# marvinli00/genie2

Hardware: AMD Instinct MI355X
Metric: denoise-steps/sec (N=256, T=1000, batch=8) (higher is better)
Workload: dtype f32 (pair-stack products as 3 f16 MFMAs on 2xf16-split operands, f32 accumulate); 1 GPU; unconditional N=256, T=1000, batch=8 per GPU, random-init base Denoiser (15.7M params), scale=0.6, reverse-loop steps 995..676; parallelism=replica per GPU x1, no data-path collective

## Files before the change

### genie2_amd/csrc/common.h

```cpp
#pragma once
#include <hip/hip_runtime.h>
#include <stdint.h>
#include "../../include/genie_hip.h"

typedef float f32x16 __attribute__((ext_vector_type(16)));
typedef float f32x4 __attribute__((ext_vector_type(4)));

#define GENIE_LN_EPS 1e-5f

#ifdef __HIPCC__

__device__ __forceinline__ f32x16 mfma_8k(const float4 a, const float4 b, f32x16 c) {
    c = __builtin_amdgcn_mfma_f32_32x32x2f32(a.x, b.x, c, 0, 0, 0);
    c = __builtin_amdgcn_mfma_f32_32x32x2f32(a.y, b.y, c, 0, 0, 0);
    c = __builtin_amdgcn_mfma_f32_32x32x2f32(a.z, b.z, c, 0, 0, 0);
    c = __builtin_amdgcn_mfma_f32_32x32x2f32(a.w, b.w, c, 0, 0, 0);
    return c;
}

__device__ __forceinline__ f32x16 zero16() {
    f32x16 z;
#pragma unroll
    for (int i = 0; i < 16; ++i) z[i] = 0.f;
    return z;
// ... 145 lines not shown
};
struct StructLayerW {
    float *proj_w, *proj_b;
    float *head_w;
    float *out_w, *out_b;
    float *ln_ipa_g, *ln_ipa_b;
    float *t1_w, *t1_b, *t2_w, *t2_b, *t3_w, *t3_b;
    float *ln_tr_g, *ln_tr_b;
    float *bb_w, *bb_b;
};

struct HxGemmW { const float* w; const unsigned char* img; float inv_s; };

struct genie_train_ws;
struct genie_ctx {
    genie_dims_t d;
    genie_train_ws* train;
    int device;
    char err[512];

    bool have_weights;
    float* wdev;
    bool hx;
    unsigned char* hxdev;
    HxGemmW hxg[128]; int n_hxg;
    unsigned hx_launches;
    size_t wdev_floats;
    float *single_w;
    float *pij_w;
    float *relpos_t;
    float *templ_w;
    float *motif_w;
    float *ipa_bias_w, *ipa_bias_b;
    PairLayerW* pair;
    StructLayerW* st;

    bool have_tables;
    float *pos_tab, *chain_tab, *t_tab, *sched;
    int n_pos, n_chain;
    float* sched_host;

    int B, N, NP;
    bool have_feats, has_motif;
    int32_t *f_aatype, *f_rmask, *f_ridx, *f_cidx;
    float *f_pos;
    uint8_t *f_fsm, *f_fstm, *f_ifm;
    float *rmaskf;

    void* ws; size_t ws_bytes;
    float *p, *acm, *bcm, *xcm, *pstatic, *ipa_bias;
    float *spart;
    unsigned *pmax;
    float *xsingle, *s0, *s, *s1, *s2, *h1, *h2, *pij, *proj, *cat;
    float *kT, *v, *qp, *kpT, *vp;
    float *vf, *vmax;
    float *ta_tb, *ta_xn, *ta_qkvg;
    float *rots_w, *trans_w;
    int32_t* tsteps;
    float *loop_z;

    bool prof;
    struct ProfRec { int cls; hipEvent_t a, b; };
    ProfRec* prof_recs; int prof_n, prof_cap;
    double prof_ms[KC_COUNT]; int64_t prof_cnt[KC_COUNT];
    double train_gemm_flop;

// ... 46 lines not shown
```

### genie2_amd/csrc/genie_api.hip

```cpp
#include <stdio.h>
#include <stdlib.h>
#include <string.h>
#include <math.h>
#include <algorithm>
#include <cmath>
#include <new>
#include <string>
#include <vector>

#include "common.h"

void pair_kernels_init();
void pair_fused_kernels_init();
void single_kernels_init(const genie_dims_t& d, int n_max);
void launch_scale_copy(genie_ctx* h, hipStream_t st, const float* in, float* out, int n, float s);
size_t ipa_attn_lds(const genie_dims_t& d, int N);

static char g_create_err[512] = "";

void set_handle_free_error(const char* msg) { snprintf(g_create_err, sizeof g_create_err, "%s", msg); }

#define SET_ERR(h, ...) do { snprintf((h)->err, sizeof((h)->err), __VA_ARGS__); } while (0)
#define HIP_TRY(h, call) do { hipError_t e_ = (call); if (e_ != hipSuccess) { \
    SET_ERR(h, "%s failed: %s (%s:%d)", #call, hipGetErrorString(e_), __FILE__, __LINE__); return GENIE_E_HIP; } } while (0)
// ... 365 lines not shown
            };
            A.sq = scale_of(q_w); A.sk = scale_of(k_w); A.sv = scale_of(v_w);
        }
        const size_t nh = (size_t)d.pair_transition_n * cp;
        const float* lg = c.take(cp); const float* lb = c.take(cp);
        const float* w1 = c.take(nh * cp); const float* b1 = c.take(nh);
        const float* w2 = c.take(cp * nh); const float* b2 = c.take(cp);
        {
            std::vector<float> w1v(w1, w1 + nh * cp), b1v(b1, b1 + nh);
            fold_ln(w1v, b1v, (int)nh, (int)cp, lg, lb);
            slot(&L.pt_ln_g, ones_off); slot(&L.pt_ln_b, zeros_off);
            slot(&L.pt_w1, img.pack(w1v.data(), (int)nh, (int)cp)); slot(&L.pt_b1, img.raw(b1v.data(), nh));
            HxTransW& X = L.hx_pt;
            const float s1 = p2floor(16384.0 / max_abs(w1v.data(), nh * cp)), s2 = p2floor(16384.0 / max_abs(w2, cp * nh));
            const float sh = p2floor(32768.0 / hx_bound(w1v.data(), b1v.data(), (int)nh, (int)cp));
            X.sx = HX_SX; X.c1 = sh / (HX_SX * s1); X.c2 = 1.0f / (sh * s2);
            hxfix.push_back({&X.img, hx.begin()});
            for (size_t hb = 0; hb < nh / 32; ++hb) {
                for (int kc = 0; kc < 8; ++kc)
                    hx.unit([&](int i, int hh, int e) { return w1v[(32 * hb + i) * cp + 16 * kc + 8 * hh + e] * s1; });
                for (int cc = 0; cc < 2; ++cc)
                    for (int ob = 0; ob < 4; ++ob)
                        hx.unit([&](int j, int hh, int e) {
                            return w2[(size_t)(32 * ob + j) * nh + 32 * hb + 16 * cc + (e & 3) + 8 * (e >> 2) + 4 * hh] * s2; });
            }
            std::vector<float> b1s(nh), b2s(cp);
            for (size_t r = 0; r < nh; ++r) b1s[r] = b1v[r] * HX_SX * s1;
            for (size_t r = 0; r < cp; ++r) b2s[r] = b2[r] * sh * s2;
            slot(&X.b1s, img.raw(b1s.data(), nh)); slot(&X.b2s, img.raw(b2s.data(), cp));
            pt_save[l] = PtSave{w1v, std::vector<float>(w2, w2 + cp * nh), s1, s2};
        }
        slot(&L.pt_w2, img.pack(w2, (int)cp, (int)nh)); slot(&L.pt_b2, img.raw(b2, cp));
    }
    {
        auto ck = [](int kc, int hh, int e) { return 16 * kc + (e & 3) + 8 * (e >> 2) + 4 * hh; };
        auto emit_O = [&](const TmSave& t) {
            for (int which = 0; which < 2; ++which)
                for (int st = 0; st < 2; ++st)
                    for (int obl = 0; obl < 2; ++obl)
                        for (int kc = 0; kc < 8; ++kc) {
                            const std::vector<float>& m = which == 0 ? t.zw : t.gw;
                            const float sc = which == 0 ? t.szo : t.sgo;
                            const size_t ob = 2 * st + obl;
                            hx.unit([&](int i, int hh, int e) { return m[(32 * ob + i) * cp + ck(kc, hh, e)] * sc; });
                        }
        };
        auto emit_T = [&](const PtSave& t) {
            const size_t nh = (size_t)d.pair_transition_n * cp;
            for (size_t hb = 0; hb < nh / 32; ++hb) {
                for (int kc = 0; kc < 8; ++kc)
                    hx.unit([&](int i, int hh, int e) { return t.w1v[(32 * hb + i) * cp + ck(kc, hh, e)] * t.s1; });
                for (int cc = 0; cc < 2; ++cc)
                    for (int ob = 0; ob < 4; ++ob)
                        hx.unit([&](int j, int hh, int e) { return t.w2[(size_t)(32 * ob + j) * nh + 32 * hb + ck(cc, hh, e)] * t.s2; });
            }
        };
        auto emit_P = [&](const TmSave& t) {
            for (size_t pass = 0; pass < 8; ++pass)
                for (int kc = 0; kc < 8; ++kc) {
                    hx.unit([&](int i, int hh, int e) { return t.w[(32 * pass + i) * cp + ck(kc, hh, e)] * t.sp; });
                    hx.unit([&](int i, int hh, int e) { return t.w[(2 * ch + 32 * pass + i) * cp + ck(kc, hh, e)] * t.sg; });
                }
        };
        for (int l = 0; l < d.n_pair_transform_layer; ++l) {
            hxfix.push_back({&h->pair[l].fa.img, hx.begin()});
            emit_O(tm_save[2 * l]); emit_P(tm_save[2 * l + 1]);
            hxfix.push_back({&h->pair[l].fb.img, hx.begin()});
            emit_O(tm_save[2 * l + 1]); emit_T(pt_save[l]);
            if (l + 1 < d.n_pair_transform_layer) emit_P(tm_save[2 * l + 2]);
        }
    }
    const size_t H = d.n_head_ipa, C = d.c_hidden_ipa, Pq = d.n_qk_point, Pv = d.n_v_point;
    const size_t ncat = ipa_cat_n(d);
    std::vector<float> wb_all, bb_all;
    for (int l = 0; l < d.n_structure_layer; ++l) {
        StructLayerW& S = h->st[l];
        const float* hw = c.take(H);
        const float* q_w = c.take(H * C * cs);            const float* q_b = c.take(H * C);
        const float* kv_w = c.take(2 * H * C * cs);       const float* kv_b = c.take(2 * H * C);
        const float* qp_w = c.take(3 * H * Pq * cs);      const float* qp_b = c.take(3 * H * Pq);
        const float* kp_w = c.take(3 * H * (Pq + Pv) * cs); const float* kp_b = c.take(3 * H * (Pq + Pv));
        const float* b_w = c.take(H * cp);                const float* b_b = c.take(H);
        const float* o_w = c.take(cs * ncat);             const float* o_b = c.take(cs);
        const float* li_g = c.take(cs); const float* li_b = c.take(cs);
        const float* t1w = c.take(cs * cs); const float* t1b = c.take(cs);
        const float* t2w = c.take(cs * cs); const float* t2b = c.take(cs);
        const float* t3w = c.take(cs * cs); const float* t3b = c.take(cs);
        const float* lt_g = c.take(cs); const float* lt_b = c.take(cs);
        const float* bw = c.take(6 * cs); const float* bbs = c.take(6);
        if (!bbs) { SET_ERR(h, "genie_load_weights: blob too short"); return GENIE_E_ARG; }
        slot(&S.head_w, img.raw(hw, H));
        auto w = vcat({{q_w, H * C * cs}, {kv_w, 2 * H * C * cs}, {qp_w, 3 * H * Pq * cs}, {kp_w, 3 * H * (Pq + Pv) * cs}});
        auto bv = vcat({{q_b, H * C}, {kv_b, 2 * H * C}, {qp_b, 3 * H * Pq}, {kp_b, 3 * H * (Pq + Pv)}});
        pack_gemm(&S.proj_w, w.data(), ipa_proj_n(d), (int)cs);
        slot(&S.proj_b, img.raw(bv.data(), bv.size()));
        wb_all.insert(wb_all.end(), b_w, b_w + H * cp);
        bb_all.insert(bb_all.end(), b_b, b_b + H);
        pack_gemm(&S.out_w, o_w, (int)cs, (int)ncat); slot(&S.out_b, img.raw(o_b, cs));
        slot(&S.ln_ipa_g, img.raw(li_g, cs)); slot(&S.ln_ipa_b, img.raw(li_b, cs));
        pack_gemm(&S.t1_w, t1w, (int)cs, (int)cs); slot(&S.t1_b, img.raw(t1b, cs));
        pack_gemm(&S.t2_w, t2w, (int)cs, (int)cs); slot(&S.t2_b, img.raw(t2b, cs));
        pack_gemm(&S.t3_w, t3w, (int)cs, (int)cs); slot(&S.t3_b, img.raw(t3b, cs));
        slot(&S.ln_tr_g, img.raw(lt_g, cs)); slot(&S.ln_tr_b, img.raw(lt_b, cs));
        slot(&S.bb_w, img.raw(bw, 6 * cs)); slot(&S.bb_b, img.raw(bbs, 6));
    }
    pack_gemm(&h->ipa_bias_w, wb_all.data(), (int)(d.n_structure_layer * H), (int)cp);
    slot(&h->ipa_bias_b, img.raw(bb_all.data(), bb_all.size()));
    if (c.left != 0) { SET_ERR(h, "genie_load_weights: %zu floats left over", c.left); return GENIE_E_ARG; }

    if (h->wdev) { (void)hipFree(h->wdev); h->wdev = nullptr; }
    img.add(64);
    HIP_TRY(h, hipMalloc((void**)&h->wdev, img.data.size() * sizeof(float)));
    HIP_TRY(h, hipMemcpy(h->wdev, img.data.data(), img.data.size() * sizeof(float), hipMemcpyHostToDevice));
    h->wdev_floats = img.data.size();
    for (auto& f : fix) *f.first = h->wdev + f.second;
    if (h->hxdev) { (void)hipFree(h->hxdev); h->hxdev = nullptr; }
    hx.begin();
    HIP_TRY(h, hipMalloc((void**)&h->hxdev, hx.d.size() * 2 + 256));
    HIP_TRY(h, hipMemcpy(h->hxdev, hx.d.data(), hx.d.size() * 2, hipMemcpyHostToDevice));
    for (auto& f : hxfix) *f.first = h->hxdev + f.second;
    h->n_hxg = 0;
    const int hxg_cap = (int)(sizeof(h->hxg) / sizeof(h->hxg[0]));
    if ((int)gfix.size() > hxg_cap) { SET_ERR(h, "genie_load_weights: %zu row-GEMM weights exceed the %d hx image slots", gfix.size(), hxg_cap); return GENIE_E_ARG; }
    for (auto& g : gfix) h->hxg[h->n_hxg++] = HxGemmW{*g.slot, h->hxdev + g.hx_off, g.inv_s};
    h->have_weights = true;
    return GENIE_OK;
}

int genie_set_tables(genie_handle_t h, const float* pos_tab, int n_pos, const float* chain_tab, int n_chain,
                     const float* t_tab, const float* sched) {
    if (!h || !pos_tab || !chain_tab || !t_tab || !sched || n_pos < 1 || n_chain < 1) return GENIE_E_ARG;
    HIP_TRY(h, hipSetDevice(h->device));
    const genie_dims_t& d = h->d;
    const size_t T1 = d.n_timestep + 1;
    const size_t a = (size_t)n_pos * d.c_pos_emb, b = (size_t)n_chain * d.c_chain_emb, c = T1 * d.c_timestep_emb, s = 4 * T1;
    if (h->pos_tab) (void)hipFree(h->pos_tab);
    HIP_TRY(h, hipMalloc((void**)&h->pos_tab, (a + b + c + s) * sizeof(float)));
    h->chain_tab = h->pos_tab + a;
    h->t_tab = h->chain_tab + b;
    h->sched = h->t_tab + c;
// ... 77 lines not shown
    HIP_TRY(h, hipMemcpyAsync(h->f_ridx, f->residue_index, M * 4, hipMemcpyDeviceToDevice, st));
    HIP_TRY(h, hipMemcpyAsync(h->f_cidx, f->chain_index, M * 4, hipMemcpyDeviceToDevice, st));
    HIP_TRY(h, hipMemcpyAsync(h->f_fsm, f->fixed_sequence_mask, M, hipMemcpyDeviceToDevice, st));
    HIP_TRY(h, hipMemcpyAsync(h->f_fstm, f->fixed_structure_mask, P, hipMemcpyDeviceToDevice, st));
    HIP_TRY(h, hipMemcpyAsync(h->f_ifm, f->interface_mask, M, hipMemcpyDeviceToDevice, st));
    hipLaunchKernelGGL(k_mask_to_float, dim3((unsigned)((M + 255) / 256)), dim3(256), 0, st, h->f_rmask, h->rmaskf, (int)M);
    HIP_TRY(h, hipMemsetAsync(h->acm, 0, (size_t)B * cp * NP * NP * 4, st));
    HIP_TRY(h, hipMemsetAsync(h->vf, 0, ipa_vf_floats(d, B, N) * 4, st));
    HIP_TRY(h, hipMemsetAsync(h->bcm, 0, (size_t)B * cp * NP * NP * 4, st));
    single_kernels_init(d, N);
    {
        unsigned any = 0;
        HIP_TRY(h, hipMemsetAsync(h->pmax, 0, sizeof(unsigned), st));
        launch_any_nonzero(h, st, h->f_fstm, P, h->pmax);
        HIP_TRY(h, hipMemcpyAsync(&any, h->pmax, sizeof(unsigned), hipMemcpyDeviceToHost, st));
        HIP_TRY(h, hipStreamSynchronize(st));
        h->has_motif = any != 0;
    }
    launch_pair_static(h, st);
    HIP_TRY(h, hipGetLastError());
    h->have_feats = true;
    return GENIE_OK;
}

static int denoise_internal(genie_ctx* h, hipStream_t st, const float* trans, const float* rots, const int32_t* ts_dev,
                            const int8_t* codes, float* z_out, const genie_taps_t* taps) {
    const genie_dims_t& d = h->d;
    const int B = h->B, N = h->N, M = B * N;
    const size_t P = (size_t)M * N;
    const int cs = d.c_s, cp = d.c_p;
    const int ldx = (single_in(d) + 7) / 8 * 8;
    auto d2d = [&](void* dst, const void* src, size_t bytes) { return hipMemcpyAsync(dst, src, bytes, hipMemcpyDeviceToDevice, st); };

    h->hx_launches = 1;
    launch_scale_copy(h, st, trans, h->trans_w, M * 3, d.rescale);
    HIP_TRY(h, d2d(h->rots_w, rots, (size_t)M * 9 * 4));

    launch_single_input(h, st, ts_dev);
    launch_gemm_rows(h, st, h->xsingle, ldx, M, ldx, h->single_w, cs, nullptr, nullptr, 0, h->rmaskf, 0, h->s0, cs);
    if (taps && taps->s) HIP_TRY(h, d2d(taps->s, h->s0, (size_t)M * cs * 4));

    launch_gemm_rows(h, st, h->s0, cs, M, cs, h->pij_w, 2 * cp, nullptr, nullptr, 0, nullptr, 0, h->pij, 2 * cp);
    launch_pair_init(h, st, h->trans_w, h->rots_w, codes);
    if (taps && taps->p_init) HIP_TRY(h, d2d(taps->p_init, h->p, P * cp * 4));

    const bool fused = launch_pair_stack_fused(h, st, taps ? taps->p_trimul_out0 : nullptr, taps ? taps->p_layer0 : nullptr);
    for (int l = 0; l < (fused ? 0 : d.n_pair_transform_layer); ++l) {
        launch_trimul(h, st, h->pair[l].out, true);
        if (l == 0 && taps && taps->p_trimul_out0) HIP_TRY(h, d2d(taps->p_trimul_out0, h->p, P * cp * 4));
        launch_trimul(h, st, h->pair[l].in, false);
        if (d.n_head_tri > 0) {
            launch_triatt(h, st, h->pair[l].ta_start, true);
            launch_triatt(h, st, h->pair[l].ta_end, false);
            if (l == 0 && taps && taps->p_tri_att0) HIP_TRY(h, d2d(taps->p_tri_att0, h->p, P * cp * 4));
        }
        launch_pair_transition(h, st, h->pair[l]);
        if (l == 0 && taps && taps->p_layer0) HIP_TRY(h, d2d(taps->p_layer0, h->p, P * cp * 4));
    }
    if (taps && taps->p) HIP_TRY(h, d2d(taps->p, h->p, P * cp * 4));

    launch_ipa_bias(h, st);
    HIP_TRY(h, d2d(h->s, h->s0, (size_t)M * cs * 4));
    if (taps && taps->states) HIP_TRY(h, d2d(taps->states, h->s0, (size_t)M * cs * 4));
    int n_state = 1;
    const int nproj = ipa_proj_n(d), ncat = ipa_cat_n(d);
    bool split = h->st2 && B >= 2 && M >= 1024 && ipa_attn_splits(h) && !getenv("GENIE_NO_STRUCT_SPLIT");
// ... 228 lines not shown
```

### genie2_amd/csrc/hx_fused.h

```cpp
#pragma once
#include "hx_pair.h"

#define FZ_SB_BZ 0
#define FZ_SB_BG 128
#define FZ_SB_B1 256
#define FZ_SB_B2 768
#define FZ_SB_BP 896
#define FZ_SB_FLOATS 1408
#define FZ_OOR 0x7FFFFFF0
#define FZ_COMPILER_FENCE() asm volatile("" ::: "memory")

struct FusedArgs {
    float* z; const float* xcm; const float* rmask; const unsigned char* wimg;
    const float *bzs, *bgs, *b1s, *b2s, *bproj;
    unsigned *acm, *bcm;
    int N, NP, n_wtiles, n_hb;
    unsigned cm_bytes, z_bytes;
    float sx, cgo, cz, c1, c2, inv_c2, cpa, cpb, cg;
    int rev;
};

__device__ __forceinline__ void fz_zt_read(float4 (&raw)[16], const unsigned char* zt, int pl, int h, int half) {
#pragma unroll
    for (int q = 0; q < 4; ++q) {
        const int g = 4 * q + h;
        raw[2 * (4 * half + q)] = *reinterpret_cast<const float4*>(zt + pl * 256 + ((g ^ (pl & 15)) << 4));
        raw[2 * (4 * half + q) + 1] = *reinterpret_cast<const float4*>(zt + pl * 256 + (((g + 2) ^ (pl & 15)) << 4));
    }
}

__device__ __forceinline__ void fz_zt_chunk(float4& a, float4& b, const unsigned char* zt, int pl, int h, int q) {
    const int g = 4 * q + h;
    a = *reinterpret_cast<const float4*>(zt + pl * 256 + ((g ^ (pl & 15)) << 4));
    b = *reinterpret_cast<const float4*>(zt + pl * 256 + (((g + 2) ^ (pl & 15)) << 4));
}

__device__ __forceinline__ void fz_store_half(rsrc_t rz, unsigned char* zt, const f32x16& v0, const f32x16& v1, int lane, int soff,
                                              int row_stride, int nvalid, int hf) {
    const int pl = lane & 31, h = lane >> 5;
    FZ_COMPILER_FENCE();
#pragma unroll
    for (int q = 0; q < 4; ++q) {
        const f32x16& v = (q < 2) ? v0 : v1;
        const int r0 = 8 * (q & 1);
        const int g = 4 * q + h;
        *reinterpret_cast<float4*>(zt + pl * 256 + ((g ^ (pl & 15)) << 4)) = make_float4(v[r0], v[r0 + 1], v[r0 + 2], v[r0 + 3]);
        *reinterpret_cast<float4*>(zt + pl * 256 + (((g + 2) ^ (pl & 15)) << 4)) = make_float4(v[r0 + 4], v[r0 + 5], v[r0 + 6], v[r0 + 7]);
    }
    hx_lds_done();
#pragma unroll
    for (int j = 0; j < 8; ++j) {
        const int r = 4 * j + (lane >> 4);
// ... 36 lines not shown
```

### genie2_amd/csrc/pair_fused_kernels.hip

```cpp
#include <string.h>
#include "hx_fused.h"

#define FZ_LDS_BYTES (2 * HX_STAGE_BYTES + 6144 + 8 * HX_ZT_BYTES)

template <bool COL, bool HAS_T, bool HAS_P = true>
__global__ __launch_bounds__(512, 1) void k_pair_fused(const FusedArgs A) {
    extern __shared__ __attribute__((aligned(16))) unsigned char smb[];
    float* sb = reinterpret_cast<float*>(smb + 2 * HX_STAGE_BYTES);
    const int lane = threadIdx.x & 63, wave = UNI(threadIdx.x >> 6);
    const int h = lane >> 5, pl = lane & 31;
    const int N = A.N, NP = A.NP, n_wtiles = A.n_wtiles;
    const int ntile = (N + 31) >> 5;
    const int n_tiles = (n_wtiles + 7) / 8;
    const int rev = A.rev;
    const int n_hb = HAS_T ? A.n_hb : 0;
    const int PBASE = 4 + n_hb;
    const rsrc_t rw = hx_rsrc(A.wimg, (unsigned)((PBASE + (HAS_P ? 8 : 0)) * HX_STAGE_BYTES));
    const rsrc_t rx = hx_rsrc(A.xcm, A.cm_bytes), rz = hx_rsrc(A.z, A.z_bytes);
    const rsrc_t ra = hx_rsrc(A.acm, A.cm_bytes), rb = hx_rsrc(A.bcm, A.cm_bytes);
    const int lane16 = lane * 16;
    const int sstride = NP * NP * 4;
    const int zstride = COL ? N * 512 : 512;
    auto issue = [&](int s, int buf) {
        if (wave >= 4) {
#pragma unroll
            for (int q = 0; q < 8; ++q) {
                const int p = 8 * (wave - 4) + q;
                hx_dma(rw, smb + buf * HX_STAGE_BYTES + p * 1024, lane16, s * HX_STAGE_BYTES + p * 1024);
            }
        }
    };
    unsigned char* zt = smb + 2 * HX_STAGE_BYTES + 6144 + wave * HX_ZT_BYTES;
    auto tile_geom = [&](int tile, int& zsoff, int& nv, int& cmoff) {
        const int wt = min(HX_PHYS(tile) * 8 + wave, n_wtiles - 1);
        const int st = wt % ntile, line = (wt / ntile) % N, b = wt / (ntile * N);
        nv = min(32, N - st * 32);
        zsoff = COL ? ((b * N + st * 32) * N + line) * 512 : ((b * N + line) * N + st * 32) * 512;
        cmoff = ((b * 128 * NP + line) * NP + st * 32) * 4;
    };
    const int vx = (4 * h * NP * NP + pl) * 4;
#define FZ_XLOAD(c, xoff) do {                                                                                              \
        raw[2 * (c)].x = hx_load(rx, vx, (xoff) + (16 * (c) + 0) * sstride); raw[2 * (c)].y = hx_load(rx, vx, (xoff) + (16 * (c) + 1) * sstride); \
        raw[2 * (c)].z = hx_load(rx, vx, (xoff) + (16 * (c) + 2) * sstride); raw[2 * (c)].w = hx_load(rx, vx, (xoff) + (16 * (c) + 3) * sstride); \
        raw[2 * (c) + 1].x = hx_load(rx, vx, (xoff) + (16 * (c) + 8) * sstride); raw[2 * (c) + 1].y = hx_load(rx, vx, (xoff) + (16 * (c) + 9) * sstride); \
        raw[2 * (c) + 1].z = hx_load(rx, vx, (xoff) + (16 * (c) + 10) * sstride); raw[2 * (c) + 1].w = hx_load(rx, vx, (xoff) + (16 * (c) + 11) * sstride); \
    } while (0)

    int tile = blockIdx.x;
    issue(0, 0);
    for (int u = threadIdx.x; u < FZ_SB_FLOATS; u += 512) {
        float v = 0.f;
        if (u < FZ_SB_BG) v = A.bzs[u];
        else if (u < FZ_SB_B1) v = A.bgs[u - FZ_SB_BG];
        else if (u < FZ_SB_B2) { if (HAS_T && u - FZ_SB_B1 < n_hb * 32) v = A.b1s[u - FZ_SB_B1]; }
        else if (u < FZ_SB_BP) { if (HAS_T) v = A.b2s[u - FZ_SB_B2]; }
        else if (HAS_P) v = A.bproj[u - FZ_SB_BP];
        sb[u] = v;
    }
    float4 raw[16];
    {
        int zs, nv, cm;
        tile_geom(tile, zs, nv, cm);
        hx_zt_dma(rz, zt, lane, zs, zstride, nv, 1);
    }
    hx_stage_landed();
    __syncthreads();

#pragma unroll 1
    for (; tile < n_tiles; tile += gridDim.x) {
        const int wt_raw = HX_PHYS(tile) * 8 + wave;
        const bool act = wt_raw < n_wtiles;
        const int wt = act ? wt_raw : n_wtiles - 1;
        const int st = wt % ntile, line = (wt / ntile) % N, b = wt / (ntile * N);
        const int t0i = st * 32;
        const int nvalid = act ? min(32, N - t0i) : 0;
        int zsoff, znv, cmoff;
        tile_geom(tile, zsoff, znv, cmoff);
        int bo = 0;
        asm volatile("" : "+v"(bo));
        const float* sbt = sb + bo;
        int lane_t = lane;
        asm volatile("" : "+v"(lane_t));
        const int pl_t = lane_t & 31, h_t = lane_t >> 5;
#pragma unroll
        for (int c = 0; c < 8; ++c) FZ_XLOAD(c, cmoff);
        const float msk = (pl < nvalid) ? A.rmask[b * N + line] * A.rmask[b * N + t0i + pl] : 0.f;
        const bool more = tile + (int)gridDim.x < n_tiles;
        int n_zsoff = 0, n_nv = 1, n_cmoff = 0;
        if (more) tile_geom(tile + gridDim.x, n_zsoff, n_nv, n_cmoff);
        hx_vm_done();
        f32x16 v[4];

// ... 89 lines not shown
                    for (int q = 0; q < 4; ++q) fz_zt_chunk(res[2 * q], res[2 * q + 1], zt, pl_t, h_t, q);
                } else {
#pragma unroll
                    for (int q = 0; q < 8; ++q) res[q] = rz1[q];
                }
#pragma unroll
                for (int r = 0; r < 16; ++r) {
                    const float g0 = A.cz * __builtin_amdgcn_rcpf(1.0f + __builtin_amdgcn_exp2f(ga[r] * A.cgo));
                    const float g1 = A.cz * __builtin_amdgcn_rcpf(1.0f + __builtin_amdgcn_exp2f(gb[r] * A.cgo));
                    const float4 za = res[2 * (r >> 3) + ((r & 7) >> 2)], zb = res[2 * (2 + (r >> 3)) + ((r & 7) >> 2)];
                    const float z0 = (r & 3) == 0 ? za.x : (r & 3) == 1 ? za.y : (r & 3) == 2 ? za.z : za.w;
                    const float z1 = (r & 3) == 0 ? zb.x : (r & 3) == 1 ? zb.y : (r & 3) == 2 ? zb.z : zb.w;
                    v[2 * half][r] = fmaf(v[2 * half][r], g0, z0);
                    v[2 * half + 1][r] = fmaf(v[2 * half + 1][r], g1, z1);
                }
                hx_stage_landed();
                hx_stage_barrier();
            }
        }

        h8 zh[8], zl[8];
        if constexpr (HAS_T) {
            float mean, sc;
            fz_stats(v, A.sx, mean, sc);
            fz_split_tile(zh, zl, v, mean, sc);
#pragma unroll
            for (int ob = 0; ob < 4; ++ob)
#pragma unroll
                for (int r = 0; r < 16; ++r) v[ob][r] = fmaf(v[ob][r], A.inv_c2, sbt[FZ_SB_B2 + ob * 32 + acc_row(r, lane)]);
            f32x16 d;
#pragma unroll
            for (int r = 0; r < 16; ++r) d[r] = sbt[FZ_SB_B1 + acc_row(r, lane)];
            auto t_stage = [&](int hb) {
                if (HAS_P || hb + 1 < n_hb) issue(4 + hb + 1, (hb + 1) & 1);
                else if (more) issue(0, 0);
                const unsigned char* stage = smb + (hb & 1) * HX_STAGE_BYTES;
                {
                    h8 wh = hx_frag(stage, 0, 0, lane), wl = hx_frag(stage, 0, 1, lane);
#pragma unroll
                    for (int kc = 0; kc < 8; ++kc) {
                        const h8 nh = hx_frag(stage, min(kc + 1, 7), 0, lane), nl = hx_frag(stage, min(kc + 1, 7), 1, lane);
                        PIPE_FENCE();
                        MFH3(wh, wl, zh[kc], zl[kc], d);
                        PIPE_FENCE();
                        wh = nh; wl = nl;
                    }
                }
                h8 ah[2], al[2];
#pragma unroll
                for (int c = 0; c < 2; ++c) {
                    float x[8];
#pragma unroll
                    for (int e = 0; e < 8; ++e) x[e] = fmaxf(d[8 * c + e], 0.f);
                    hx_split8(x, A.c1, ah[c], al[c]);
                }
                {
                    h8 bh = hx_frag(stage, 8, 0, lane), bl = hx_frag(stage, 8, 1, lane);
#pragma unroll
                    for (int u = 0; u < 8; ++u) {
                        const h8 nh = hx_frag(stage, 8 + min(u + 1, 7), 0, lane), nl = hx_frag(stage, 8 + min(u + 1, 7), 1, lane);
                        PIPE_FENCE();
                        MFH3(bh, bl, ah[u >> 2], al[u >> 2], v[u & 3]);
                        PIPE_FENCE();
                        bh = nh; bl = nl;
                        if (u == 1) {
#pragma unroll
                            for (int r = 0; r < 16; ++r) d[r] = sbt[FZ_SB_B1 + (hb + 1) * 32 + acc_row(r, lane)];
                        }
                    }
                }
                hx_stage_landed();
                hx_stage_barrier();
            };
#pragma unroll 1
            for (int hb = 0; hb < n_hb; ++hb) t_stage(hb);
            const float m2 = msk * A.c2;
#pragma unroll
            for (int ob = 0; ob < 4; ++ob)
#pragma unroll
                for (int r = 0; r < 16; ++r) v[ob][r] *= m2;
        }

        fz_store_half(rz, zt, v[0], v[1], lane_t, zsoff, zstride, nvalid, 0);
        FZ_COMPILER_FENCE();
        fz_store_half(rz, zt, v[2], v[3], lane_t, zsoff, zstride, nvalid, 1);
        FZ_COMPILER_FENCE();
        if constexpr (HAS_P) {
            float mean, sc;
            fz_stats(v, A.sx, mean, sc);
            fz_split_tile(zh, zl, v, mean, sc);
        }
        hx_lds_done();
        if constexpr (!HAS_P) {
            if (more) hx_zt_dma(rz, zt, lane_t, n_zsoff, zstride, n_nv, 1);
        }

        if constexpr (HAS_P) {
            const float* sbias = sbt + FZ_SB_BP;
            const float cg = A.cg;
            const float ma = msk * A.cpa, mb = msk * A.cpb;
            const int voff = (pl < nvalid) ? (4 * h * NP * NP + pl) * 4 : FZ_OOR;
            const int sbase = ((b * 128 * NP + line) * NP + t0i) * 4;
            unsigned wst[8];
            f32x16 apA, agA, apB, agB;
#pragma unroll
            for (int r = 0; r < 16; ++r) { apB[r] = 0.f; agB[r] = 0.f; apA[r] = sbias[acc_row(r, lane)]; agA[r] = sbias[256 + acc_row(r, lane)]; }
#pragma unroll 1
            for (int pp = 0; pp < 4; ++pp) {
                {
                    const int pass = 2 * pp;
                    issue(PBASE + pass + 1, 1);
                    const unsigned char* stage = smb;
                    const rsrc_t e_rd = pp > 2 ? rb : ra;
                    const int e_voff = pp == 0 ? FZ_OOR : voff;
                    const int e_so = sbase + ((pass - 1) & 3) * 32 * sstride;
                    const float e_pm = pp > 2 ? mb : ma;
                    HX_PROJ_STAGE(apA, agA, apB, agB);
                    asm volatile("s_waitcnt vmcnt(16)" ::: "memory");
                    if (more) {
                        if (pp == 2) hx_zt_dma(rz, zt, lane_t, n_zsoff, zstride, n_nv, 1, 0, 4);
                    }
                    hx_stage_barrier();
                }
                {
                    const int pass = 2 * pp + 1;
                    if (pp < 3) issue(PBASE + pass + 1, 0);
                    else if (more) issue(0, 0);
                    const unsigned char* stage = smb + HX_STAGE_BYTES;
                    const rsrc_t e_rd = pp < 2 ? ra : rb;
                    const int e_voff = voff;
                    const int e_so = sbase + ((pass - 1) & 3) * 32 * sstride;
                    const float e_pm = pp < 2 ? ma : mb;
                    HX_PROJ_STAGE(apB, agB, apA, agA);
                    asm volatile("s_waitcnt vmcnt(16)" ::: "memory");
                    if (more) {
                        if (pp == 2) hx_zt_dma(rz, zt, lane_t, n_zsoff, zstride, n_nv, 1, 4, 4);
                    }
                    hx_stage_barrier();
                }
            }
            {
                const rsrc_t e_rd = rb;
                const int e_voff = voff, e_so = sbase + 3 * 32 * sstride;
                const float e_pm = mb;
                float t[16], u[16];
#pragma unroll
                for (int r = 0; r < 16; ++r) {
                    HX_PROJ_PIECE_A(agB, r, t[r]);
                    HX_PROJ_PIECE_B(apB, r, t[r], u[r]);
                }
                PIPE_FENCE();
#pragma unroll
                for (int r = 0; r < 16; ++r) HX_PROJ_PIECE_C_NOW(r, t[r], u[r]);
            }
        }
    }
#undef FZ_XLOAD
}

static int fz_num_cu() {
    static int n = 0;
    if (!n) { int dev = 0; hipDeviceProp_t pr; (void)hipGetDevice(&dev); (void)hipGetDeviceProperties(&pr, dev); n = pr.multiProcessorCount > 0 ? pr.multiProcessorCount : 256; }
    return n;
}

void pair_fused_kernels_init() {
    (void)hipFuncSetAttribute(reinterpret_cast<const void*>(k_pair_fused<true, false>), hipFuncAttributeMaxDynamicSharedMemorySize, FZ_LDS_BYTES);
    (void)hipFuncSetAttribute(reinterpret_cast<const void*>(k_pair_fused<false, true>), hipFuncAttributeMaxDynamicSharedMemorySize, FZ_LDS_BYTES);
    (void)hipFuncSetAttribute(reinterpret_cast<const void*>(k_pair_fused<false, true, false>), hipFuncAttributeMaxDynamicSharedMemorySize, FZ_LDS_BYTES);
}

void launch_pair_fused(genie_ctx* h, hipStream_t st, const HxFusedW& f, const HxTriW& o, const HxTransW* t, const HxTriW* pp, bool col) {
    const HxTriW& p = pp ? *pp : o;
    const int N = h->N, NP = h->NP, ntile = (N + 31) / 32;
    FusedArgs a;
    a.z = h->p; a.xcm = h->xcm; a.rmask = h->rmaskf; a.wimg = f.img;
    a.bzs = o.bzs; a.bgs = o.bgs; a.b1s = t ? t->b1s : nullptr; a.b2s = t ? t->b2s : nullptr; a.bproj = p.bias_proj;
    a.acm = reinterpret_cast<unsigned*>(h->acm); a.bcm = reinterpret_cast<unsigned*>(h->bcm);
    a.N = N; a.NP = NP; a.n_wtiles = h->B * N * ntile; a.n_hb = t ? h->d.pair_transition_n * 4 : 0;
    a.cm_bytes = (unsigned)((size_t)h->B * 128 * NP * NP * 4);
    a.z_bytes = (unsigned)((size_t)h->B * N * N * 512);
    a.sx = o.sx; a.cgo = o.cgo; a.cz = o.cz;
    a.c1 = t ? t->c1 : 0.f; a.c2 = t ? t->c2 : 1.f; a.inv_c2 = t ? 1.0f / t->c2 : 1.f;
    a.cpa = p.cpa; a.cpb = p.cpb; a.cg = p.cg;
    a.rev = (int)(h->hx_launches++ & 1);
    const long long n_tiles = ((long long)a.n_wtiles + 7) / 8;
    const unsigned grid = (unsigned)(n_tiles < fz_num_cu() ? n_tiles : fz_num_cu());
    if (!pp) hipLaunchKernelGGL((k_pair_fused<false, true, false>), dim3(grid), dim3(512), FZ_LDS_BYTES, st, a);
    else if (col) hipLaunchKernelGGL((k_pair_fused<true, false>), dim3(grid), dim3(512), FZ_LDS_BYTES, st, a);
    else hipLaunchKernelGGL((k_pair_fused<false, true>), dim3(grid), dim3(512), FZ_LDS_BYTES, st, a);
}
```

### genie2_amd/csrc/pair_hx_kernels.hip

```cpp
#include "hx_pair.h"


template <int NW>
__global__ __launch_bounds__(NW * 64, NW == 8 ? 1 : 2) void k_pair_transition_hx(
    float* __restrict__ z, const float* __restrict__ rmask, const unsigned char* __restrict__ wimg,
    const float* __restrict__ b1s, const float* __restrict__ b2s, int N, long long M, int n_hb, float sx, float c1, float c2, int rev) {
    extern __shared__ __attribute__((aligned(16))) unsigned char smb[];
    float* sb1 = reinterpret_cast<float*>(smb + 2 * HX_STAGE_BYTES);
    const int lane = threadIdx.x & 63, wave = UNI(threadIdx.x >> 6);
    const int h = lane >> 5, pl = lane & 31;
    const int n_wt = (int)((M + 31) / 32);
    const int n_tiles = (n_wt + NW - 1) / NW;
    const rsrc_t rw = hx_rsrc(wimg, (unsigned)(n_hb * HX_STAGE_BYTES));
    const rsrc_t rz = hx_rsrc(z, (unsigned)(M * 512));
    const rsrc_t rnull = hx_rsrc(z, 0u);
    const int lane16 = lane * 16;
    constexpr int PW = 32 / NW;
    auto issue = [&](int hb, int buf) {
#pragma unroll
        for (int q = 0; q < PW; ++q) {
            const int p = PW * wave + q;
            hx_dma(rw, smb + buf * HX_STAGE_BYTES + p * 1024, lane16, hb * HX_STAGE_BYTES + p * 1024);
        }
    };
// ... 688 lines not shown
    const unsigned* bcm = reinterpret_cast<const unsigned*>(h->bcm);
    const unsigned* pa = transposed ? bcm : acm;
    const unsigned* pb = transposed ? acm : bcm;
    if (g.NP > 192 && g.NP <= 256) {
        hipLaunchKernelGGL(k_trimul_contract_hx_big, dim3(BC < ncu ? BC : ncu), dim3(512), 4 * CB_PLANE, st, pa, pb, h->xcm, g.NP, BC, g.cm_bytes,
                           x.cx, rev);
    } else if (g.NP >= 128) {
        const int tiles = (g.NP + 127) / 128;
        const int n_tiles = tiles * tiles * ((BC + 7) / 8) * 8;
        hipLaunchKernelGGL(k_trimul_contract_hx<2>, dim3(n_tiles < 3 * ncu ? n_tiles : 3 * ncu), dim3(256), 2 * 4 * 128 * CX_ROWB, st,
                           pa, pb, h->xcm, g.NP, BC, g.cm_bytes, x.cx, rev);
    } else {
        const int tiles = (g.NP + 63) / 64;
        const int n_tiles = tiles * tiles * ((BC + 7) / 8) * 8;
        hipLaunchKernelGGL(k_trimul_contract_hx<1>, dim3(n_tiles < 4 * ncu ? n_tiles : 4 * ncu), dim3(256), 2 * 4 * 64 * CX_ROWB, st,
                           pa, pb, h->xcm, g.NP, BC, g.cm_bytes, x.cx, rev);
    }
}

static void hx_trimul_out(genie_ctx* h, hipStream_t st, const TriMulW& w) {
    const HxTriGeom g = tri_geom(h);
    const HxTriW& x = w.hx;
    ProfScope ps(h, st, KC_TRIMUL_OUT);
    hipLaunchKernelGGL(k_trimul_out_hx_r<8>, dim3(hx_grid((g.n_wt + 7) / 8, 8)), dim3(512), 4 * HX_STAGE_BYTES, st, h->p, h->xcm,
                       x.img_out, x.bgs, x.bzs, g.N, g.NP, g.n_wt, g.cm_bytes, g.z_bytes, x.sx, x.cgo, x.cz, (int)(h->hx_launches++ & 1));
}

void launch_trimul_hx(genie_ctx* h, hipStream_t st, const TriMulW& w, bool outgoing) {
    hx_trimul_proj(h, st, w, outgoing);
    hx_trimul_contract(h, st, w, false);
    hx_trimul_out(h, st, w);
}

void launch_pair_fused(genie_ctx* h, hipStream_t st, const HxFusedW& f, const HxTriW& o, const HxTransW* t, const HxTriW* p, bool col);
bool launch_pair_stack_fused(genie_ctx* h, hipStream_t st, float* tap_trimul_out0, float* tap_layer0) {
    const int L = h->d.n_pair_transform_layer;
    if (!h->hx || L < 1 || getenv("GENIE_NO_PAIR_FUSE")) return false;
    if (h->d.n_head_tri > 0) return false;
    const size_t pbytes = (size_t)h->B * h->N * h->N * h->d.c_p * 4;
    hx_trimul_proj(h, st, h->pair[0].out, true);
    for (int l = 0; l < L; ++l) {
        const PairLayerW& W = h->pair[l];
        hx_trimul_contract(h, st, W.out, true);
        { ProfScope ps(h, st, KC_PAIR_FUSED_A); launch_pair_fused(h, st, W.fa, W.out.hx, nullptr, &W.in.hx, true); }
        if (l == 0 && tap_trimul_out0) (void)hipMemcpyAsync(tap_trimul_out0, h->p, pbytes, hipMemcpyDeviceToDevice, st);
        hx_trimul_contract(h, st, W.in, false);
        {
            ProfScope ps(h, st, KC_PAIR_FUSED_B);
            launch_pair_fused(h, st, W.fb, W.in.hx, &W.hx_pt, l + 1 < L ? &h->pair[l + 1].out.hx : nullptr, false);
        }
        if (l == 0 && tap_layer0) (void)hipMemcpyAsync(tap_layer0, h->p, pbytes, hipMemcpyDeviceToDevice, st);
    }
    return true;
}


#define IB_UNITS 24
__global__ __launch_bounds__(256) void k_ipa_bias_hx(const float* __restrict__ z, const unsigned char* __restrict__ wimg, float inv_sw,
                                                     const float* __restrict__ bias, float* __restrict__ out, int B, int N, int LH,
                                                     int n_tiles, int rev, unsigned* pmax) {
    extern __shared__ __attribute__((aligned(16))) unsigned char ibw[];
    float* sbias = reinterpret_cast<float*>(ibw + IB_UNITS * 2048);
    const int tid = threadIdx.x, lane = tid & 63, wave = tid >> 6;
    for (int u = tid; u < IB_UNITS * 128; u += 256) reinterpret_cast<uint4*>(ibw)[u] = reinterpret_cast<const uint4*>(wimg)[u];
    if (tid < 96) sbias[tid] = tid < LH ? bias[tid] : 0.f;
    __syncthreads();
    const int n = lane & 31, hf = lane >> 5;
    const int jt = (N + 31) >> 5;
    float amax = 0.f;
    for (int t = blockIdx.x * 4 + wave; t < n_tiles; t += gridDim.x * 4) {
        const int tt = rev ? n_tiles - 1 - t : t;
        const int j0 = (tt % jt) * 32;
        const int bi = tt / jt;
        const int j = min(j0 + n, N - 1);
        const float* row = z + ((size_t)bi * N + j) * 128 + 8 * hf;
        float4 x[8][2];
#pragma unroll
        for (int s = 0; s < 8; ++s) {
            x[s][0] = *reinterpret_cast<const float4*>(row + 16 * s);
            x[s][1] = *reinterpret_cast<const float4*>(row + 16 * s + 4);
        }
        float m = 0.f;
// ... 68 lines not shown
```

### genie2_amd/csrc/pair_kernels.hip

```cpp
#include "common.h"

#define LDZ 132


template <bool AMAX = false>
__device__ __forceinline__ float load_tile64(float* tile, const float* __restrict__ src, size_t row_stride,
                                             int nvalid, int tid) {
    const int c4 = tid & 31;
    const int r0 = tid >> 5;
    float4 v[8];
    const int last = max(nvalid - 1, 0);
#pragma unroll
    for (int u = 0; u < 8; ++u) {
        const int r = min(r0 + 8 * u, last);
        v[u] = *reinterpret_cast<const float4*>(src + (size_t)r * row_stride + c4 * 4);
    }
#pragma unroll
    for (int u = 0; u < 8; ++u) {
        const int r = r0 + 8 * u;
        if (r >= nvalid) v[u] = make_float4(0.f, 0.f, 0.f, 0.f);
        *reinterpret_cast<float4*>(tile + r * LDZ + c4 * 4) = v[u];
    }
    float am = 0.f;
    if constexpr (AMAX) {
// ... 398 lines not shown
        const int BC = h->B * h->d.c_hidden_mul;
        const unsigned cm_bytes = (unsigned)((size_t)BC * NP * NP * 4);
        static int num_cu = 0;
        if (!num_cu) { int dev = 0; hipDeviceProp_t pr; (void)hipGetDevice(&dev); (void)hipGetDeviceProperties(&pr, dev); num_cu = pr.multiProcessorCount > 0 ? pr.multiProcessorCount : 256; }
        if (NP >= 128) {
            const int tiles = (NP + 127) / 128;
            const int n_tiles = tiles * tiles * ((BC + 7) / 8) * 8;
            const size_t lds = 2 * 2 * 128 * LDK * sizeof(float);
            hipLaunchKernelGGL(k_trimul_contract<2>, dim3(n_tiles < 2 * num_cu ? n_tiles : 2 * num_cu), dim3(256), lds, st, h->acm,
                               h->bcm, h->xcm, NP, BC, cm_bytes);
        } else {
            const int tiles = (NP + 63) / 64;
            const int n_tiles = tiles * tiles * ((BC + 7) / 8) * 8;
            const size_t lds = 2 * 2 * 64 * LDK * sizeof(float);
            hipLaunchKernelGGL(k_trimul_contract<1>, dim3(n_tiles < 4 * num_cu ? n_tiles : 4 * num_cu), dim3(256), lds, st, h->acm,
                               h->bcm, h->xcm, NP, BC, cm_bytes);
        }
    }
    {
        ProfScope ps(h, st, KC_TRIMUL_OUT);
        launch_trimul_out_wl(h, st, w);
    }
}

void launch_pair_transition_hx(genie_ctx* h, hipStream_t st, const PairLayerW& w);
void launch_pair_transition(genie_ctx* h, hipStream_t st, const PairLayerW& w) {
    ProfScope ps(h, st, KC_PAIR_TRANSITION);
    if (h->hx) launch_pair_transition_hx(h, st, w);
    else launch_pair_transition_wl(h, st, w);
}

bool launch_ipa_bias_hx(genie_ctx* h, hipStream_t st);
void launch_ipa_bias(genie_ctx* h, hipStream_t st) {
    ProfScope ps(h, st, KC_IPA_BIAS);
    if (launch_ipa_bias_hx(h, st)) return;
    const int N = h->N, ntile = (N + 127) / 128;
    const int LH = h->d.n_structure_layer * h->d.n_head_ipa;
    const size_t lds = 128 * LDZ * sizeof(float);
    (void)hipMemsetAsync(h->pmax, 0, sizeof(unsigned), st);
    hipLaunchKernelGGL(k_ipa_bias, dim3(h->B * N * ntile), dim3(256), lds, st, h->p, h->ipa_bias_w, h->ipa_bias_b, h->ipa_bias,
                       h->B, N, LH, h->hx ? (int)(h->hx_launches & 1) : 0, h->pmax);
}

void pair_wl_kernels_init();
void pair_hx_kernels_init();
void pair_kernels_init() {
    pair_wl_kernels_init();
    pair_hx_kernels_init();
    (void)hipFuncSetAttribute(reinterpret_cast<const void*>(k_trimul_contract<2>), hipFuncAttributeMaxDynamicSharedMemorySize,
                        2 * 2 * 128 * LDK * sizeof(float));
    (void)hipFuncSetAttribute(reinterpret_cast<const void*>(k_ipa_bias), hipFuncAttributeMaxDynamicSharedMemorySize,
                        128 * LDZ * sizeof(float));
}
```

Baseline: 111.1 batch-steps/s.

## Fuse IPA pair-bias projection into the last pair-stack fused kernel

Computes the IPA attention bias (pair rep projected to all layers' heads) inside the final fused pair kernel while the tile is still in registers, instead of rereading the full pair tensor in a separate ipa_bias kernel. Bias weights are packed as extra hx stages with their own power-of-two scale, and the pair abs-max is reduced with an atomicMax into pmax. The cost is extra MFMA work and stores in the last fused kernel, plus more register pressure and weight staging there.

Measured after the change: 111.9 batch-steps/s, median of 6. No clear change (+0.7%).

```diff
diff --git a/genie2_amd/csrc/common.h b/genie2_amd/csrc/common.h
--- a/genie2_amd/csrc/common.h
+++ b/genie2_amd/csrc/common.h
@@ -201,6 +201,8 @@
     float *templ_w;
     float *motif_w;
     float *ipa_bias_w, *ipa_bias_b;
+    bool ib_fused; float ib_inv_s;
+    bool ib_done;
     PairLayerW* pair;
     StructLayerW* st;
 
diff --git a/genie2_amd/csrc/genie_api.hip b/genie2_amd/csrc/genie_api.hip
--- a/genie2_amd/csrc/genie_api.hip
+++ b/genie2_amd/csrc/genie_api.hip
@@ -421,7 +421,8 @@
         }
         slot(&L.pt_w2, img.pack(w2, (int)cp, (int)nh)); slot(&L.pt_b2, img.raw(b2, cp));
     }
-    {
+    std::vector<float> wb_all, bb_all;
+    auto emit_fused_chains = [&]() {
         auto ck = [](int kc, int hh, int e) { return 16 * kc + (e & 3) + 8 * (e >> 2) + 4 * hh; };
         auto emit_O = [&](const TmSave& t) {
             for (int which = 0; which < 2; ++which)
@@ -458,10 +459,19 @@
             emit_O(tm_save[2 * l + 1]); emit_T(pt_save[l]);
             if (l + 1 < d.n_pair_transform_layer) emit_P(tm_save[2 * l + 2]);
         }
-    }
+        const int LH = (int)(d.n_structure_layer * d.n_head_ipa);
+        h->ib_fused = d.n_pair_transform_layer > 0 && LH <= 96 && cp == 128;
+        if (h->ib_fused) {
+            const float sw = p2floor(16384.0 / max_abs(wb_all.data(), wb_all.size()));
+            h->ib_inv_s = 1.0f / sw;
+            for (int u = 0; u < 32; ++u)
+                hx.unit([&](int i, int hh, int e) {
+                    const int r = 32 * (u >> 3) + i;
+                    return (u < 24 && r < LH) ? wb_all[(size_t)r * cp + ck(u & 7, hh, e)] * sw : 0.f; });
+        }
+    };
     const size_t H = d.n_head_ipa, C = d.c_hidden_ipa, Pq = d.n_qk_point, Pv = d.n_v_point;
     const size_t ncat = ipa_cat_n(d);
-    std::vector<float> wb_all, bb_all;
     for (int l = 0; l < d.n_structure_layer; ++l) {
         StructLayerW& S = h->st[l];
         const float* hw = c.take(H);
@@ -495,6 +505,7 @@
     }
     pack_gemm(&h->ipa_bias_w, wb_all.data(), (int)(d.n_structure_layer * H), (int)cp);
     slot(&h->ipa_bias_b, img.raw(bb_all.data(), bb_all.size()));
+    emit_fused_chains();
     if (c.left != 0) { SET_ERR(h, "genie_load_weights: %zu floats left over", c.left); return GENIE_E_ARG; }
 
     if (h->wdev) { (void)hipFree(h->wdev); h->wdev = nullptr; }
@@ -638,6 +649,7 @@
     const int ldx = (single_in(d) + 7) / 8 * 8;
     auto d2d = [&](void* dst, const void* src, size_t bytes) { return hipMemcpyAsync(dst, src, bytes, hipMemcpyDeviceToDevice, st); };
 
+    h->ib_done = false;
     h->hx_launches = 1;
     launch_scale_copy(h, st, trans, h->trans_w, M * 3, d.rescale);
     HIP_TRY(h, d2d(h->rots_w, rots, (size_t)M * 9 * 4));
diff --git a/genie2_amd/csrc/hx_fused.h b/genie2_amd/csrc/hx_fused.h
--- a/genie2_amd/csrc/hx_fused.h
+++ b/genie2_amd/csrc/hx_fused.h
@@ -18,6 +18,9 @@
     unsigned cm_bytes, z_bytes;
     float sx, cgo, cz, c1, c2, inv_c2, cpa, cpb, cg;
     int rev;
+    float* ib_out; const float* ib_b; unsigned* pmax;
+    unsigned ib_bytes; int ib_ostride, LH;
+    float ib_inv_sw;
 };
 
 __device__ __forceinline__ void fz_zt_read(float4 (&raw)[16], const unsigned char* zt, int pl, int h, int half) {
diff --git a/genie2_amd/csrc/pair_fused_kernels.hip b/genie2_amd/csrc/pair_fused_kernels.hip
--- a/genie2_amd/csrc/pair_fused_kernels.hip
+++ b/genie2_amd/csrc/pair_fused_kernels.hip
@@ -3,8 +3,9 @@
 
 #define FZ_LDS_BYTES (2 * HX_STAGE_BYTES + 6144 + 8 * HX_ZT_BYTES)
 
-template <bool COL, bool HAS_T, bool HAS_P = true>
+template <bool COL, bool HAS_T, bool HAS_P = true, bool HAS_BIAS = false>
 __global__ __launch_bounds__(512, 1) void k_pair_fused(const FusedArgs A) {
+    static_assert(!HAS_BIAS || (!HAS_P && HAS_T && !COL), "the pair bias leaves with the last chain");
     extern __shared__ __attribute__((aligned(16))) unsigned char smb[];
     float* sb = reinterpret_cast<float*>(smb + 2 * HX_STAGE_BYTES);
     const int lane = threadIdx.x & 63, wave = UNI(threadIdx.x >> 6);
@@ -15,7 +16,7 @@
     const int rev = A.rev;
     const int n_hb = HAS_T ? A.n_hb : 0;
     const int PBASE = 4 + n_hb;
-    const rsrc_t rw = hx_rsrc(A.wimg, (unsigned)((PBASE + (HAS_P ? 8 : 0)) * HX_STAGE_BYTES));
+    const rsrc_t rw = hx_rsrc(A.wimg, (unsigned)((PBASE + (HAS_P ? 8 : HAS_BIAS ? 2 : 0)) * HX_STAGE_BYTES));
     const rsrc_t rx = hx_rsrc(A.xcm, A.cm_bytes), rz = hx_rsrc(A.z, A.z_bytes);
     const rsrc_t ra = hx_rsrc(A.acm, A.cm_bytes), rb = hx_rsrc(A.bcm, A.cm_bytes);
     const int lane16 = lane * 16;
@@ -55,9 +56,11 @@
         else if (u < FZ_SB_B2) { if (HAS_T && u - FZ_SB_B1 < n_hb * 32) v = A.b1s[u - FZ_SB_B1]; }
         else if (u < FZ_SB_BP) { if (HAS_T) v = A.b2s[u - FZ_SB_B2]; }
         else if (HAS_P) v = A.bproj[u - FZ_SB_BP];
+        else if (HAS_BIAS) { if (u - FZ_SB_BP < A.LH) v = A.ib_b[u - FZ_SB_BP]; }
         sb[u] = v;
     }
     float4 raw[16];
+    float amax = 0.f;
     {
         int zs, nv, cm;
         tile_geom(tile, zs, nv, cm);
@@ -213,7 +216,7 @@
 #pragma unroll
             for (int r = 0; r < 16; ++r) d[r] = sbt[FZ_SB_B1 + acc_row(r, lane)];
             auto t_stage = [&](int hb) {
-                if (HAS_P || hb + 1 < n_hb) issue(4 + hb + 1, (hb + 1) & 1);
+                if (HAS_P || HAS_BIAS || hb + 1 < n_hb) issue(4 + hb + 1, (hb + 1) & 1);
                 else if (more) issue(0, 0);
                 const unsigned char* stage = smb + (hb & 1) * HX_STAGE_BYTES;
                 {
@@ -274,6 +277,72 @@
         hx_lds_done();
         if constexpr (!HAS_P) {
             if (more) hx_zt_dma(rz, zt, lane_t, n_zsoff, zstride, n_nv, 1);
+        }
+
+        if constexpr (HAS_BIAS) {
+            float m = 0.f;
+#pragma unroll
+            for (int ob = 0; ob < 4; ++ob)
+#pragma unroll
+                for (int r = 0; r < 16; ++r) m = fmaxf(m, fabsf(v[ob][r]));
+            m = fmaxf(m, __shfl_xor(m, 32));
+            amax = fmaxf(amax, m);
+            const int ex = (int)((__builtin_bit_cast(unsigned, m) >> 23) & 255u);
+            const bool tiny = ex < 16;
+            const float sc = tiny ? 1.0f : __builtin_bit_cast(float, (unsigned)(268 - ex) << 23);
+            const float isc = (tiny ? 1.0f : __builtin_bit_cast(float, (unsigned)(ex - 14) << 23)) * A.ib_inv_sw;
+            fz_split_tile(zh, zl, v, 0.f, sc);
+            const rsrc_t ro = hx_rsrc(A.ib_out, A.ib_bytes);
+            const int ostride = A.ib_ostride;
+            const int obase = ((b * N + line) * N + t0i) * 4;
+            const float* sib = sbt + FZ_SB_BP;
+            auto bias_store = [&](const f32x16& acc, int blk, int r) {
+                const int rc = (r & 3) + 8 * (r >> 2);
+                const int voff = (pl < nvalid && 32 * blk + rc + 4 * h < A.LH) ? 4 * h * ostride + pl * 4 : FZ_OOR;
+                hx_store(ro, fmaf(acc[r], isc, sib[32 * blk + rc + 4 * h_t]), voff, obase + (32 * blk + rc) * ostride);
+            };
+            f32x16 b0, b1, b2;
+#pragma unroll
+            for (int r = 0; r < 16; ++r) { b0[r] = 0.f; b1[r] = 0.f; b2[r] = 0.f; }
+            {
+                issue(PBASE + 1, 1);
+                const unsigned char* stage = smb;
+                h8 f0 = hx_frag(stage, 0, 0, lane), f0l = hx_frag(stage, 0, 1, lane), f1 = hx_frag(stage, 8, 0, lane),
+                   f1l = hx_frag(stage, 8, 1, lane);
+#pragma unroll
+                for (int kc = 0; kc < 8; ++kc) {
+                    const int kn = min(kc + 1, 7);
+                    const h8 n0 = hx_frag(stage, kn, 0, lane), n0l = hx_frag(stage, kn, 1, lane), n1 = hx_frag(stage, 8 + kn, 0, lane),
+                             n1l = hx_frag(stage, 8 + kn, 1, lane);
+                    PIPE_FENCE();
+                    MFH3(f0, f0l, zh[kc], zl[kc], b0);
+                    MFH3(f1, f1l, zh[kc], zl[kc], b1);
+                    PIPE_FENCE();
+                    f0 = n0; f0l = n0l; f1 = n1; f1l = n1l;
+                }
+                hx_stage_landed();
+                hx_stage_barrier();
+            }
+            {
+                if (more) issue(0, 0);
+                const unsigned char* stage = smb + HX_STAGE_BYTES;
+                h8 f0 = hx_frag(stage, 0, 0, lane), f0l = hx_frag(stage, 0, 1, lane);
+#pragma unroll
+                for (int kc = 0; kc < 8; ++kc) {
+                    const int kn = min(kc + 1, 7);
+                    const h8 n0 = hx_frag(stage, kn, 0, lane), n0l = hx_frag(stage, kn, 1, lane);
+                    PIPE_FENCE();
+                    MFH3(f0, f0l, zh[kc], zl[kc], b2);
+                    PIPE_FENCE();
+                    f0 = n0; f0l = n0l;
+                    bias_store(b0, 0, 2 * kc); bias_store(b0, 0, 2 * kc + 1);
+                    bias_store(b1, 1, 2 * kc); bias_store(b1, 1, 2 * kc + 1);
+                }
+                hx_stage_landed();
+                hx_stage_barrier();
+#pragma unroll
+                for (int r = 0; r < 16; ++r) bias_store(b2, 2, r);
+            }
         }
 
         if constexpr (HAS_P) {
@@ -336,6 +405,11 @@
             }
         }
     }
+    if constexpr (HAS_BIAS) {
+#pragma unroll
+        for (int o = 32; o > 0; o >>= 1) amax = fmaxf(amax, __shfl_xor(amax, o));
+        if (lane == 0 && __float_as_uint(amax) > *reinterpret_cast<volatile unsigned*>(A.pmax)) atomicMax(A.pmax, __float_as_uint(amax));
+    }
 #undef FZ_XLOAD
 }
 
@@ -349,9 +423,10 @@
     (void)hipFuncSetAttribute(reinterpret_cast<const void*>(k_pair_fused<true, false>), hipFuncAttributeMaxDynamicSharedMemorySize, FZ_LDS_BYTES);
     (void)hipFuncSetAttribute(reinterpret_cast<const void*>(k_pair_fused<false, true>), hipFuncAttributeMaxDynamicSharedMemorySize, FZ_LDS_BYTES);
     (void)hipFuncSetAttribute(reinterpret_cast<const void*>(k_pair_fused<false, true, false>), hipFuncAttributeMaxDynamicSharedMemorySize, FZ_LDS_BYTES);
+    (void)hipFuncSetAttribute(reinterpret_cast<const void*>(k_pair_fused<false, true, false, true>), hipFuncAttributeMaxDynamicSharedMemorySize, FZ_LDS_BYTES);
 }
 
-void launch_pair_fused(genie_ctx* h, hipStream_t st, const HxFusedW& f, const HxTriW& o, const HxTransW* t, const HxTriW* pp, bool col) {
+void launch_pair_fused(genie_ctx* h, hipStream_t st, const HxFusedW& f, const HxTriW& o, const HxTransW* t, const HxTriW* pp, bool col, bool bias) {
     const HxTriW& p = pp ? *pp : o;
     const int N = h->N, NP = h->NP, ntile = (N + 31) / 32;
     FusedArgs a;
@@ -365,9 +440,15 @@
     a.c1 = t ? t->c1 : 0.f; a.c2 = t ? t->c2 : 1.f; a.inv_c2 = t ? 1.0f / t->c2 : 1.f;
     a.cpa = p.cpa; a.cpb = p.cpb; a.cg = p.cg;
     a.rev = (int)(h->hx_launches++ & 1);
+    a.LH = h->d.n_structure_layer * h->d.n_head_ipa;
+    a.ib_out = h->ipa_bias; a.ib_b = h->ipa_bias_b; a.pmax = h->pmax; a.ib_inv_sw = h->ib_inv_s;
+    a.ib_ostride = h->B * N * N * 4; a.ib_bytes = (unsigned)((size_t)a.LH * a.ib_ostride);
     const long long n_tiles = ((long long)a.n_wtiles + 7) / 8;
     const unsigned grid = (unsigned)(n_tiles < fz_num_cu() ? n_tiles : fz_num_cu());
-    if (!pp) hipLaunchKernelGGL((k_pair_fused<false, true, false>), dim3(grid), dim3(512), FZ_LDS_BYTES, st, a);
+    if (!pp && bias) {
+        (void)hipMemsetAsync(h->pmax, 0, sizeof(unsigned), st);
+        hipLaunchKernelGGL((k_pair_fused<false, true, false, true>), dim3(grid), dim3(512), FZ_LDS_BYTES, st, a);
+    } else if (!pp) hipLaunchKernelGGL((k_pair_fused<false, true, false>), dim3(grid), dim3(512), FZ_LDS_BYTES, st, a);
     else if (col) hipLaunchKernelGGL((k_pair_fused<true, false>), dim3(grid), dim3(512), FZ_LDS_BYTES, st, a);
     else hipLaunchKernelGGL((k_pair_fused<false, true>), dim3(grid), dim3(512), FZ_LDS_BYTES, st, a);
 }
diff --git a/genie2_amd/csrc/pair_hx_kernels.hip b/genie2_amd/csrc/pair_hx_kernels.hip
--- a/genie2_amd/csrc/pair_hx_kernels.hip
+++ b/genie2_amd/csrc/pair_hx_kernels.hip
@@ -744,7 +744,7 @@
     hx_trimul_out(h, st, w);
 }
 
-void launch_pair_fused(genie_ctx* h, hipStream_t st, const HxFusedW& f, const HxTriW& o, const HxTransW* t, const HxTriW* p, bool col);
+void launch_pair_fused(genie_ctx* h, hipStream_t st, const HxFusedW& f, const HxTriW& o, const HxTransW* t, const HxTriW* p, bool col, bool bias);
 bool launch_pair_stack_fused(genie_ctx* h, hipStream_t st, float* tap_trimul_out0, float* tap_layer0) {
     const int L = h->d.n_pair_transform_layer;
     if (!h->hx || L < 1 || getenv("GENIE_NO_PAIR_FUSE")) return false;
@@ -754,12 +754,14 @@
     for (int l = 0; l < L; ++l) {
         const PairLayerW& W = h->pair[l];
         hx_trimul_contract(h, st, W.out, true);
-        { ProfScope ps(h, st, KC_PAIR_FUSED_A); launch_pair_fused(h, st, W.fa, W.out.hx, nullptr, &W.in.hx, true); }
+        { ProfScope ps(h, st, KC_PAIR_FUSED_A); launch_pair_fused(h, st, W.fa, W.out.hx, nullptr, &W.in.hx, true, false); }
         if (l == 0 && tap_trimul_out0) (void)hipMemcpyAsync(tap_trimul_out0, h->p, pbytes, hipMemcpyDeviceToDevice, st);
         hx_trimul_contract(h, st, W.in, false);
         {
             ProfScope ps(h, st, KC_PAIR_FUSED_B);
-            launch_pair_fused(h, st, W.fb, W.in.hx, &W.hx_pt, l + 1 < L ? &h->pair[l + 1].out.hx : nullptr, false);
+            const bool bias = l + 1 == L && h->ib_fused;
+            launch_pair_fused(h, st, W.fb, W.in.hx, &W.hx_pt, l + 1 < L ? &h->pair[l + 1].out.hx : nullptr, false, bias);
+            if (bias) h->ib_done = true;
         }
         if (l == 0 && tap_layer0) (void)hipMemcpyAsync(tap_layer0, h->p, pbytes, hipMemcpyDeviceToDevice, st);
     }
diff --git a/genie2_amd/csrc/pair_kernels.hip b/genie2_amd/csrc/pair_kernels.hip
--- a/genie2_amd/csrc/pair_kernels.hip
+++ b/genie2_amd/csrc/pair_kernels.hip
@@ -454,6 +454,7 @@
 
 bool launch_ipa_bias_hx(genie_ctx* h, hipStream_t st);
 void launch_ipa_bias(genie_ctx* h, hipStream_t st) {
+    if (h->ib_done) return;
     ProfScope ps(h, st, KC_IPA_BIAS);
     if (launch_ipa_bias_hx(h, st)) return;
     const int N = h->N, ntile = (N + 127) / 128;
```
